# ZrrSkywalker/MonoDETR

Measured on AMD Instinct MI355X. Metric: training images/sec at B=8 per GPU, KITTI 384x1280, higher is better.
Workload: dtype bf16; 1 GPU; full MonoDETR training step (ResNet-50 + depth predictor + 3 enc / 3 dec layers, 550 train queries, 4 levels, criterion + AdamW) = BASELINE configs[2] (1 GPU) / configs[3] (DDP); global_batch=8, per_gpu_batch=8, image=3x384x1280, queries=50, precision=bf16, parallelism=dp1, grad_sync=none, prime_steps=12, launch=one hipGraph replay per iteration, cpu_affinity=NUMA node 0 of the GPU

## Files before the change

monodetr_amd/csrc/add_ln.hip:

```cpp
#include <hip/hip_runtime.h>
#include <hip/hip_bf16.h>
#include <stdint.h>

#include "add_ln.h"
#include "add_ln_math.h"

namespace mdetr {
namespace {

constexpr int kWavesLn = 4;
constexpr int kMaxBwdBlocks = 1024;

template <typename T> __device__ __forceinline__ float ld1(const T *p);
template <> __device__ __forceinline__ float ld1<float>(const float *p) { return *p; }
template <> __device__ __forceinline__ float ld1<__hip_bfloat16>(const __hip_bfloat16 *p) { return __bfloat162float(*p); }
template <typename T> __device__ __forceinline__ void st1(T *p, float v);
template <> __device__ __forceinline__ void st1<float>(float *p, float v) { *p = v; }
template <> __device__ __forceinline__ void st1<__hip_bfloat16>(__hip_bfloat16 *p, float v) { *p = __float2bfloat16(v); }

template <typename T, int E> struct alignas(sizeof(T) * E > 16 ? 16 : sizeof(T) * E) RowVec { T v[E]; };

template <typename T, int E> __device__ __forceinline__ void load_row(const T *p, float (&v)[E])
{
    const RowVec<T, E> t = *reinterpret_cast<const RowVec<T, E> *>(p);
#pragma unroll
    for (int i = 0; i < E; ++i) v[i] = ld1<T>(&t.v[i]);
}
template <typename T, int E> __device__ __forceinline__ void store_row(T *p, const float (&v)[E])
{
    RowVec<T, E> t;
#pragma unroll
    for (int i = 0; i < E; ++i) st1<T>(&t.v[i], v[i]);
    *reinterpret_cast<RowVec<T, E> *>(p) = t;
}

__device__ __forceinline__ float wave_sum(float v)
{
#pragma unroll
    for (int o = 32; o > 0; o >>= 1) v += __shfl_xor(v, o);
    return v;
}

template <typename T, typename PT, int E>
__global__ __launch_bounds__(kWavesLn * 64)
void add_ln_fwd_kernel(const T *__restrict__ a, const T *__restrict__ b, const PT *__restrict__ gamma,
                       const PT *__restrict__ beta, T *__restrict__ y, T *__restrict__ s, float *__restrict__ stats,
                       int64_t rows, float eps, uint32_t thresh, float keep_scale, uint64_t seed,
                       const uint64_t *__restrict__ seed_dev)
{
    constexpr int C = 64 * E;
    const int lane = threadIdx.x & 63, wave = threadIdx.x >> 6;
    const int64_t row = static_cast<int64_t>(blockIdx.x) * kWavesLn + wave;
    if (row >= rows) return;
    const uint64_t sd = seed + (seed_dev ? *seed_dev : 0ull);
    const int64_t at = row * C + lane * E;
    float v[E];
    load_row<T, E>(a + at, v);
    if (b) {
        float r[E];
        load_row<T, E>(b + at, r);
#pragma unroll
        for (int i = 0; i < E; ++i) {
            const bool keep = thresh == 0u || ln_hash(sd, static_cast<uint64_t>(at + i)) >= thresh;
            v[i] += keep ? r[i] * keep_scale : 0.f;
        }
        if (s) {
            store_row<T, E>(s + at, v);
#pragma unroll
            for (int i = 0; i < E; ++i) { T t; st1<T>(&t, v[i]); v[i] = ld1<T>(&t); }
        }
    }
    float sum = 0.f;
#pragma unroll
    for (int i = 0; i < E; ++i) sum += v[i];
    const float mean = wave_sum(sum) * (1.0f / C);
    float sq = 0.f;
#pragma unroll
    for (int i = 0; i < E; ++i) { const float d = v[i] - mean; sq += d * d; }
    const float rstd = 1.0f / sqrtf(wave_sum(sq) * (1.0f / C) + eps);
    float o[E];
#pragma unroll
    for (int i = 0; i < E; ++i) o[i] = (v[i] - mean) * rstd * ld1<PT>(gamma + lane * E + i) + ld1<PT>(beta + lane * E + i);
    store_row<T, E>(y + at, o);
    if (lane == 0) { stats[2 * row] = mean; stats[2 * row + 1] = rstd; }
}

template <typename T, typename PT, int E>
__global__ __launch_bounds__(kWavesLn * 64)
void add_ln_bwd_kernel(const T *__restrict__ dy, const T *__restrict__ s, const PT *__restrict__ gamma,
                       const float *__restrict__ stats, T *__restrict__ da, T *__restrict__ db,
                       float *__restrict__ partial, int64_t rows, uint32_t thresh, float keep_scale, uint64_t seed,
                       const uint64_t *__restrict__ seed_dev)
{
    constexpr int C = 64 * E;
    __shared__ float red[kWavesLn][2 * C];
    const int lane = threadIdx.x & 63, wave = threadIdx.x >> 6;
    const uint64_t sd = seed + (seed_dev ? *seed_dev : 0ull);
    float g[E], acc_g[E], acc_b[E];
#pragma unroll
    for (int i = 0; i < E; ++i) { g[i] = ld1<PT>(gamma + lane * E + i); acc_g[i] = 0.f; acc_b[i] = 0.f; }
    for (int64_t row = static_cast<int64_t>(blockIdx.x) * kWavesLn + wave; row < rows; row += static_cast<int64_t>(gridDim.x) * kWavesLn) {
        const int64_t at = row * C + lane * E;
        const float mean = stats[2 * row], rstd = stats[2 * row + 1];
        float d[E], x[E];
        load_row<T, E>(dy + at, d);
        load_row<T, E>(s + at, x);
        float s1 = 0.f, s2 = 0.f;
#pragma unroll
        for (int i = 0; i < E; ++i) {
            x[i] = (x[i] - mean) * rstd;
            acc_g[i] += d[i] * x[i];
            acc_b[i] += d[i];
            d[i] *= g[i];
            s1 += d[i];
            s2 += d[i] * x[i];
        }
        s1 = wave_sum(s1) * (1.0f / C);
        s2 = wave_sum(s2) * (1.0f / C);
        float o[E];
#pragma unroll
        for (int i = 0; i < E; ++i) o[i] = rstd * (d[i] - s1 - x[i] * s2);
        store_row<T, E>(da + at, o);
        if (db) {
#pragma unroll
            for (int i = 0; i < E; ++i) {
                const bool keep = thresh == 0u || ln_hash(sd, static_cast<uint64_t>(at + i)) >= thresh;
                o[i] = keep ? o[i] * keep_scale : 0.f;
            }
            store_row<T, E>(db + at, o);
        }
    }
#pragma unroll
    for (int i = 0; i < E; ++i) { red[wave][lane * E + i] = acc_g[i]; red[wave][C + lane * E + i] = acc_b[i]; }
    __syncthreads();
    for (int c = threadIdx.x; c < 2 * C; c += kWavesLn * 64)
        partial[static_cast<int64_t>(blockIdx.x) * 2 * C + c] = red[0][c] + red[1][c] + red[2][c] + red[3][c];
}

template <typename T, typename PT, int E>
hipError_t launch_fwd(const AddLnProblem &p, const void *a, const void *b, const void *gamma, const void *beta, void *y, void *s,
                      float *stats, hipStream_t st)
{
    const uint32_t thresh = b ? ln_threshold(p.dropout_p) : 0u;
    const float scale = p.dropout_p > 0.f ? 1.0f / (1.0f - p.dropout_p) : 1.0f;
    hipLaunchKernelGGL((add_ln_fwd_kernel<T, PT, E>), dim3(static_cast<unsigned>((p.rows + kWavesLn - 1) / kWavesLn)), dim3(kWavesLn * 64), 0, st,
                       static_cast<const T *>(a), static_cast<const T *>(b), static_cast<const PT *>(gamma), static_cast<const PT *>(beta),
                       static_cast<T *>(y), static_cast<T *>(s), stats,
                       p.rows, p.eps, thresh, scale, p.seed, p.seed_dev);
    return hipGetLastError();
}

template <typename T, typename PT, int E>
hipError_t launch_bwd(const AddLnProblem &p, const void *dy, const void *s, const void *gamma, const float *stats, void *da, void *db,
                      float *partial, hipStream_t st)
{
    const uint32_t thresh = db ? ln_threshold(p.dropout_p) : 0u;
    const float scale = p.dropout_p > 0.f ? 1.0f / (1.0f - p.dropout_p) : 1.0f;
    hipLaunchKernelGGL((add_ln_bwd_kernel<T, PT, E>), dim3(static_cast<unsigned>(add_ln_partial_rows(p.rows))), dim3(kWavesLn * 64), 0, st,
                       static_cast<const T *>(dy), static_cast<const T *>(s), static_cast<const PT *>(gamma), stats, static_cast<T *>(da),
                       static_cast<T *>(db), partial,
                       p.rows, thresh, scale, p.seed, p.seed_dev);
    return hipGetLastError();
}

}

int64_t add_ln_partial_rows(int64_t rows)
{
    const int64_t blocks = (rows + kWavesLn - 1) / kWavesLn;
    return blocks < 1 ? 1 : (blocks > kMaxBwdBlocks ? kMaxBwdBlocks : blocks);
}

template <int E>
hipError_t dispatch_fwd(const AddLnProblem &p, const void *a, const void *b, const void *gamma, const void *beta, void *y, void *s,
                        float *stats, hipStream_t st)
{
    using BF = __hip_bfloat16;
    if (p.io_dtype == 2) return p.param_dtype == 2 ? launch_fwd<BF, BF, E>(p, a, b, gamma, beta, y, s, stats, st) : launch_fwd<BF, float, E>(p, a, b, gamma, beta, y, s, stats, st);
    return p.param_dtype == 2 ? launch_fwd<float, BF, E>(p, a, b, gamma, beta, y, s, stats, st) : launch_fwd<float, float, E>(p, a, b, gamma, beta, y, s, stats, st);
}

template <int E>
hipError_t dispatch_bwd(const AddLnProblem &p, const void *dy, const void *s, const void *gamma, const float *stats, void *da, void *db,
                        float *partial, hipStream_t st)
{
    using BF = __hip_bfloat16;
    if (p.io_dtype == 2) return p.param_dtype == 2 ? launch_bwd<BF, BF, E>(p, dy, s, gamma, stats, da, db, partial, st) : launch_bwd<BF, float, E>(p, dy, s, gamma, stats, da, db, partial, st);
    return p.param_dtype == 2 ? launch_bwd<float, BF, E>(p, dy, s, gamma, stats, da, db, partial, st) : launch_bwd<float, float, E>(p, dy, s, gamma, stats, da, db, partial, st);
}

hipError_t add_ln_forward_launch(const AddLnProblem &p, const void *a, const void *b, const void *gamma, const void *beta,
                                 void *y, void *s, float *stats, hipStream_t st)
{
    if (p.rows == 0) return hipSuccess;
    switch (p.cols) {
    case 128: return dispatch_fwd<2>(p, a, b, gamma, beta, y, s, stats, st);
    case 256: return dispatch_fwd<4>(p, a, b, gamma, beta, y, s, stats, st);
    case 512: return dispatch_fwd<8>(p, a, b, gamma, beta, y, s, stats, st);
    default: return hipErrorNotSupported;
    }
}

hipError_t add_ln_backward_launch(const AddLnProblem &p, const void *dy, const void *s, const void *gamma, const float *stats,
                                  void *da, void *db, float *partial, hipStream_t st)
{
    if (p.rows == 0) return hipSuccess;
    switch (p.cols) {
    case 128: return dispatch_bwd<2>(p, dy, s, gamma, stats, da, db, partial, st);
    case 256: return dispatch_bwd<4>(p, dy, s, gamma, stats, da, db, partial, st);
    case 512: return dispatch_bwd<8>(p, dy, s, gamma, stats, da, db, partial, st);
    default: return hipErrorNotSupported;
    }
}

}
```

monodetr_amd/csrc/add_ln_math.h:

```cpp
#pragma once
#include <stdint.h>

#if defined(__HIPCC__)
#define MDETR_HD __host__ __device__ __forceinline__
#else
#define MDETR_HD inline
#endif

namespace mdetr {

MDETR_HD uint32_t ln_hash(uint64_t seed, uint64_t index)
{
    uint64_t z = index * 0x9E3779B97F4A7C15ull + seed;
    uint32_t x = static_cast<uint32_t>(z) ^ static_cast<uint32_t>(z >> 32);
    x ^= x >> 16;
    x *= 0x7FEB352Du;
    x ^= x >> 15;
    x *= 0x846CA68Bu;
    x ^= x >> 16;
    return x;
}

MDETR_HD uint32_t ln_threshold(float p)
{
    const double t = static_cast<double>(p) * 4294967296.0;
    return t >= 4294967295.0 ? 0xFFFFFFFFu : static_cast<uint32_t>(t);
}

}
```

monodetr_amd/csrc/conv_wgrad.hip:

```cpp
#include <hip/hip_runtime.h>
#include <stdint.h>
#include <stdlib.h>

#include <mdetr_wave.h>

#include "conv_wgrad.h"
#include "mdetr_tune.h"
#include "mdetr_transpose.h"
#include "mdetr_split.h"
#include "msda.h"

namespace mdetr {
namespace {

constexpr int kThreadsG = 512;
constexpr int kNB = 128, kCB = 64;
#ifndef MDETR_CONV_WGRAD_COLS
#define MDETR_CONV_WGRAD_COLS 16
#endif
constexpr int kRows = 8, kCols = MDETR_CONV_WGRAD_COLS;
constexpr int kDyStride = kCols + 1;

struct WgradGeom {
    ConvWgradDims d;
    int bands, ctiles, units, chunks, nblocks, cblocks;
};

template <int SI, int TS>
__global__ __launch_bounds__(kThreadsG)
void conv_wgrad_kernel(const __bf16 *__restrict__ x, const __bf16 *__restrict__ dy, float *__restrict__ part, const WgradGeom g)
{
    constexpr int P = TS == 3 ? 1 : 0;
    constexpr int XC = SI == 1 ? kCols + TS - 1 : (TS == 3 ? 2 * kCols + 1 : kCols);
    constexpr int XSTRIDE = XC | 1;
    constexpr int EVEN = kCols + 1;
    MDETR_DYNAMIC_LDS(unsigned char, wgrad_smem);
    bf16x8 *dyt = reinterpret_cast<bf16x8 *>(wgrad_smem);
    bf16x8 *xt = dyt + kNB * kDyStride;
    const ConvWgradDims &d = g.d;
    const int lane = threadIdx.x & 63, wave = threadIdx.x >> 6, half = lane >> 5, l31 = lane & 31;
    const int nsub = wave & 3, csub = wave >> 2;
    int id = blockIdx.x;
    const int chunk = id % g.chunks; id /= g.chunks;
    const int t = id % TS; id /= TS;
    const int cblk = id % g.cblocks; const int nblk = id / g.cblocks;
    const int n0 = nblk * kNB, c0 = cblk * kCB;

    f32x16 acc[TS];
#pragma unroll
    for (int e = 0; e < TS; ++e)
#pragma unroll
        for (int i = 0; i < 16; ++i) acc[e][i] = 0.f;
    const bool want_db = TS == 1 && d.DB != 0 && cblk == 0 && csub == 0;
    f32x16 accb;
#pragma unroll
    for (int i = 0; i < 16; ++i) accb[i] = 0.f;
    bf16x8 ones;
#pragma unroll
    for (int i = 0; i < 8; ++i) ones[i] = static_cast<__bf16>(1.0f);

    constexpr int CGX = (XC + 15) / 16;
    constexpr int WTASKS = 2 * CGX + 4 * (kCols / 16);
    constexpr int kWavesG = kThreadsG / 64;
    constexpr int ROUNDS = (WTASKS + kWavesG - 1) / kWavesG;
    constexpr int PF = ROUNDS <= 2 ? 2 : 1;
    bf16x8 stage[PF][ROUNDS][8];
    const mdetr_rsrc xr = make_rsrc(x, static_cast<unsigned>(static_cast<int64_t>(d.B) * d.H * d.W * d.C * 2));
    const mdetr_rsrc yr = make_rsrc(dy, static_cast<unsigned>(static_cast<int64_t>(d.B) * d.OH * d.OW * d.N * 2));
    const int ci = lane & 15, pi = lane >> 4;
    int t_rel[ROUNDS], t_ch[ROUNDS], t_dst[ROUNDS];
#pragma unroll
    for (int rd = 0; rd < ROUNDS; ++rd) {
        const int wt = wave + rd * kWavesG;
        if (wt < 2 * CGX) {
            const int slot = 16 * (wt >> 1) + ci, piece = 4 * (wt & 1) + pi;
            t_rel[rd] = slot >= XC ? -1 : (SI == 1 ? slot : (TS == 3 ? (slot < EVEN ? 2 * slot : 2 * (slot - EVEN) + 1) : 2 * slot));
            t_ch[rd] = (c0 + piece * 8) * 2;
            t_dst[rd] = piece * 8 * XSTRIDE + slot;
        } else {
            const int k = wt - 2 * CGX, col = 16 * (k >> 2) + ci, piece = 4 * (k & 3) + pi;
            t_rel[rd] = col;
            t_ch[rd] = (wt < WTASKS && n0 + piece * 8 < d.N) ? (n0 + piece * 8) * 2 : -1;
            t_dst[rd] = piece * 8 * kDyStride + col;
        }
    }
    auto fetch = [&](int u, bf16x8 (&st)[ROUNDS][8]) {
        const int ct = u % g.ctiles; u /= g.ctiles;
        const int band = u % g.bands; const int b = u / g.bands;
        const int r0 = band * kRows, q0 = ct * kCols;
#pragma unroll
        for (int rd = 0; rd < ROUNDS; ++rd) {
            const int wt = wave + rd * kWavesG;
            if (wt < 2 * CGX) {
                const int col = SI * q0 + t_rel[rd] - P;
                const unsigned lane_off = (t_rel[rd] >= 0 && col >= 0 && col < d.W) ? static_cast<unsigned>(col * d.C * 2 + t_ch[rd]) : kRsrcOob;
#pragma unroll
                for (int i = 0; i < 8; ++i) {
                    const int row = SI * (r0 + i) + t - P;
                    const bool ok = row >= 0 && row < d.H;
                    st[rd][i] = rsrc_load_bf16x8(xr, ok ? lane_off : kRsrcOob, ok ? static_cast<unsigned>((b * d.H + row) * d.W) * static_cast<unsigned>(d.C * 2) : 0u);
                }
            } else if (wt < WTASKS) {
                const int col = q0 + t_rel[rd];
                const unsigned lane_off = (col < d.OW && t_ch[rd] >= 0) ? static_cast<unsigned>(col * d.N * 2 + t_ch[rd]) : kRsrcOob;
#pragma unroll
                for (int i = 0; i < 8; ++i) {
                    const int row = r0 + i;
                    const bool ok = row < d.OH;
                    st[rd][i] = rsrc_load_bf16x8(yr, ok ? lane_off : kRsrcOob, ok ? static_cast<unsigned>((b * d.OH + row) * d.OW) * static_cast<unsigned>(d.N * 2) : 0u);
                }
            }
        }
    };
    auto commit = [&](const bf16x8 (&st)[ROUNDS][8]) {
#pragma unroll
        for (int rd = 0; rd < ROUNDS; ++rd) {
            const int wt = wave + rd * kWavesG;
            if (wt >= WTASKS) continue;
            bf16x8 tr[8];
            transpose8x8(st[rd], tr);
            if (wt < 2 * CGX) {
                if (16 * (wt >> 1) + ci < XC) {
#pragma unroll
                    for (int q = 0; q < 8; ++q) xt[t_dst[rd] + q * XSTRIDE] = tr[q];
                }
            } else {
#pragma unroll
                for (int q = 0; q < 8; ++q) dyt[t_dst[rd] + q * kDyStride] = tr[q];
            }
        }
    };
    auto products = [&]() {
        const bf16x8 *ap = dyt + (nsub * 32 + l31) * kDyStride + half;
        const bf16x8 *bp = xt + (csub * 32 + l31) * XSTRIDE;
#pragma unroll 4
        for (int ks = 0; ks < kCols / 2; ++ks) {
            const int q = 2 * ks + half;
            const bf16x8 a = ap[2 * ks];
#pragma unroll
            for (int e = 0; e < TS; ++e) {
                int slot;
                if (SI == 1) slot = q + e;
                else if (TS == 3) slot = (e & 1) ? EVEN + q : q + (e >> 1);
                else slot = q;
                acc[e] = mfma_bf16(a, bp[slot], acc[e]);
            }
            if (want_db) accb = mfma_bf16(a, ones, accb);
        }
    };

    int u = chunk;
    if (u < g.units) fetch(u, stage[0]);
    if (PF == 2 && u + g.chunks < g.units) fetch(u + g.chunks, stage[PF - 1]);
    while (u < g.units) {
#pragma unroll
        for (int s_ = 0; s_ < PF; ++s_) {
            if (u >= g.units) break;
            __syncthreads();
            commit(stage[s_]);
            const int nu = u + PF * g.chunks;
            if (nu < g.units) fetch(nu, stage[s_]);
            __syncthreads();
            products();
            u += g.chunks;
        }
    }

    const int c = c0 + csub * 32 + l31;
    float *pp = part + static_cast<int64_t>(chunk) * (static_cast<int64_t>(d.N) * TS * TS * d.C + (d.DB ? d.N : 0));
    if (want_db && l31 == 0) {
#pragma unroll
        for (int r = 0; r < 16; ++r) {
            const int n = n0 + nsub * 32 + (r & 3) + 8 * (r >> 2) + 4 * half;
            if (n < d.N) pp[static_cast<int64_t>(d.N) * d.C + n] = accb[r];
        }
    }
#pragma unroll
    for (int e = 0; e < TS; ++e)
#pragma unroll
        for (int r = 0; r < 16; ++r) {
            const int n = n0 + nsub * 32 + (r & 3) + 8 * (r >> 2) + 4 * half;
            if (n < d.N) pp[((static_cast<int64_t>(n) * TS + t) * TS + e) * d.C + c] = acc[e][r];
        }
}

template <int SI, int TS>
hipError_t launch(const void *x, const void *dy, float *part, WgradGeom g, hipStream_t st)
{
    constexpr int XC = SI == 1 ? kCols + TS - 1 : (TS == 3 ? 2 * kCols + 1 : kCols);
    constexpr size_t lds = (static_cast<size_t>(kNB) * kDyStride + static_cast<size_t>(kCB) * (XC | 1)) * 16;
    static_assert(lds <= 160 * 1024, "tile does not fit the LDS");
    auto kern = conv_wgrad_kernel<SI, TS>;
    static bool attr_set[64] = {};
    int dev_ = 0;
    if (hipGetDevice(&dev_) != hipSuccess) dev_ = -1;
    if (dev_ < 0 || dev_ >= 64 || !attr_set[dev_]) {
        const hipError_t e = hipFuncSetAttribute(reinterpret_cast<const void *>(kern), hipFuncAttributeMaxDynamicSharedMemorySize,
                                                 static_cast<int>(lds));
        if (e != hipSuccess) return e;
        if (dev_ >= 0 && dev_ < 64) attr_set[dev_] = true;
    }
    const int64_t blocks = static_cast<int64_t>(g.chunks) * TS * g.cblocks * g.nblocks;
    hipLaunchKernelGGL(kern, dim3(static_cast<unsigned>(blocks)), dim3(kThreadsG), lds, st, static_cast<const __bf16 *>(x),
                       static_cast<const __bf16 *>(dy), part, g);
    return hipGetLastError();
}

constexpr int kCols32 = 16;
constexpr int kDyStride32 = kCols32 + 1, kXC32 = kCols32 + 2, kXStride32 = kXC32 | 1;
constexpr int kDyPlane32 = kNB * kDyStride32, kXPlane32 = kCB * kXStride32;
constexpr size_t kLds32 = static_cast<size_t>(3) * (kDyPlane32 + kXPlane32) * 16;
static_assert(kLds32 == 162816 && kLds32 <= 160 * 1024, "three planes of the 128 x 64 tile: one workgroup per CU");

__global__ __launch_bounds__(kThreadsG)
void conv_wgrad_f32_kernel(const float *__restrict__ x, const float *__restrict__ dy, float *__restrict__ part, const WgradGeom g)
{
    constexpr int TS = 3;
    MDETR_DYNAMIC_LDS(unsigned char, wgrad32_smem);
    bf16x8 *dyt = reinterpret_cast<bf16x8 *>(wgrad32_smem);
    bf16x8 *xt = dyt + 3 * kDyPlane32;
    const ConvWgradDims &d = g.d;
    const int lane = threadIdx.x & 63, wave = threadIdx.x >> 6, half = lane >> 5, l31 = lane & 31;
    const int nsub = wave & 3, csub = wave >> 2;
    int id = blockIdx.x;
    const int chunk = id % g.chunks; id /= g.chunks;
    const int t = id % TS; id /= TS;
    const int cblk = id % g.cblocks; const int nblk = id / g.cblocks;
    const int n0 = nblk * kNB, c0 = cblk * kCB;

    f32x16 acc[TS];
#pragma unroll
    for (int e = 0; e < TS; ++e)
#pragma unroll
        for (int i = 0; i < 16; ++i) acc[e][i] = 0.f;

    constexpr int CGX = (kXC32 + 15) / 16;
    constexpr int WTASKS = 2 * CGX + 4 * (kCols32 / 16);
    static_assert(WTASKS == kThreadsG / 64, "one loading task per wave");
    bf16x8 stage[16];
    const mdetr_rsrc xr = make_rsrc(x, static_cast<unsigned>(static_cast<int64_t>(d.B) * d.H * d.W * d.C * 4));
    const mdetr_rsrc yr = make_rsrc(dy, static_cast<unsigned>(static_cast<int64_t>(d.B) * d.OH * d.OW * d.N * 4));
    const int ci = lane & 15, pi = lane >> 4;
    const bool is_x = wave < 2 * CGX;
    int t_rel, t_ch, t_dst;
    if (is_x) {
        const int slot = 16 * (wave >> 1) + ci, piece = 4 * (wave & 1) + pi;
        t_rel = slot >= kXC32 ? -1 : slot;
        t_ch = (c0 + piece * 8) * 4;
        t_dst = piece * 8 * kXStride32 + slot;
    } else {
        const int k = wave - 2 * CGX, col = 16 * (k >> 2) + ci, piece = 4 * (k & 3) + pi;
        t_rel = col;
        t_ch = n0 + piece * 8 < d.N ? (n0 + piece * 8) * 4 : -1;
        t_dst = piece * 8 * kDyStride32 + col;
    }
    auto fetch = [&](int u) {
        const int ct = u % g.ctiles; u /= g.ctiles;
        const int band = u % g.bands; const int b = u / g.bands;
        const int r0 = band * kRows, q0 = ct * kCols32;
        if (is_x) {
            const int col = q0 + t_rel - 1;
            const bool in = t_rel >= 0 && col >= 0 && col < d.W;
            const unsigned lane_off = in ? static_cast<unsigned>(col * d.C * 4 + t_ch) : 0u;
#pragma unroll
            for (int i = 0; i < 8; ++i) {
                const int row = r0 + i + t - 1;
                const bool ok = in && row >= 0 && row < d.H;
                const unsigned so = (row >= 0 && row < d.H) ? static_cast<unsigned>((b * d.H + row) * d.W) * static_cast<unsigned>(d.C * 4) : 0u;
                stage[2 * i] = rsrc_load_bf16x8(xr, ok ? lane_off : kRsrcOob, so);
                stage[2 * i + 1] = rsrc_load_bf16x8(xr, ok ? lane_off + 16u : kRsrcOob, so);
            }
        } else {
            const int col = q0 + t_rel;
            const bool in = col < d.OW && t_ch >= 0;
            const unsigned lane_off = in ? static_cast<unsigned>(col * d.N * 4 + t_ch) : 0u;
#pragma unroll
            for (int i = 0; i < 8; ++i) {
                const int row = r0 + i;
                const bool ok = in && row < d.OH;
                const unsigned so = row < d.OH ? static_cast<unsigned>((b * d.OH + row) * d.OW) * static_cast<unsigned>(d.N * 4) : 0u;
                stage[2 * i] = rsrc_load_bf16x8(yr, ok ? lane_off : kRsrcOob, so);
                stage[2 * i + 1] = rsrc_load_bf16x8(yr, ok ? lane_off + 16u : kRsrcOob, so);
            }
        }
    };
    auto commit = [&]() {
        bf16x8 pl[3][8];
#pragma unroll
        for (int i = 0; i < 8; ++i) {
#pragma unroll
            for (int s = 0; s < 2; ++s) {
                float f[4];
                __builtin_memcpy(f, &stage[2 * i + s], 16);
                bf16x4 h, m, l;
                split4(f, h, m, l);
#pragma unroll
                for (int j = 0; j < 4; ++j) { pl[0][i][4 * s + j] = h[j]; pl[1][i][4 * s + j] = m[j]; pl[2][i][4 * s + j] = l[j]; }
            }
        }
        if (is_x && t_rel < 0) return;
        bf16x8 *dst = is_x ? xt + t_dst : dyt + t_dst;
        const int stride = is_x ? kXStride32 : kDyStride32, plane = is_x ? kXPlane32 : kDyPlane32;
#pragma unroll
        for (int p = 0; p < 3; ++p) {
            bf16x8 tr[8];
            transpose8x8(pl[p], tr);
#pragma unroll
            for (int q = 0; q < 8; ++q) dst[p * plane + q * stride] = tr[q];
        }
    };
    auto products = [&]() {
        const bf16x8 *ap = dyt + (nsub * 32 + l31) * kDyStride32 + half;
        const bf16x8 *bp = xt + (csub * 32 + l31) * kXStride32 + half;
        constexpr int term_y[6] = {2, 0, 1, 1, 0, 0}, term_x[6] = {0, 2, 1, 0, 1, 0};
#pragma unroll 2
        for (int ks = 0; ks < kCols32 / 2; ++ks) {
            bf16x8 a[3], b[TS][3];
#pragma unroll
            for (int p = 0; p < 3; ++p) {
                a[p] = ap[p * kDyPlane32 + 2 * ks];
#pragma unroll
                for (int e = 0; e < TS; ++e) b[e][p] = bp[p * kXPlane32 + 2 * ks + e];
            }
#pragma unroll
            for (int k = 0; k < 6; ++k)
#pragma unroll
                for (int e = 0; e < TS; ++e) acc[e] = mfma_bf16(a[term_y[k]], b[e][term_x[k]], acc[e]);
        }
    };

    int u = chunk;
    if (u < g.units) fetch(u);
    while (u < g.units) {
        __syncthreads();
        commit();
        const int nu = u + g.chunks;
        if (nu < g.units) fetch(nu);
        __syncthreads();
        products();
        u = nu;
    }

    const int c = c0 + csub * 32 + l31;
    float *pp = part + static_cast<int64_t>(chunk) * (static_cast<int64_t>(d.N) * TS * TS * d.C);
#pragma unroll
// ... 51 lines not shown
#pragma unroll
    for (int e = 0; e < TS; ++e)
#pragma unroll
        for (int i = 0; i < 16; ++i) acc[e][i] = 0.f;

    constexpr int CGX = (kXCS2 + 7) / 8;
    static_assert(CGX + 1 == kThreadsS2 / 64, "one loading task per wave");
    bf16x8 stage[16];
    const mdetr_rsrc xr = make_rsrc(x, static_cast<unsigned>(static_cast<int64_t>(d.B) * d.H * d.W * d.C * 4));
    const mdetr_rsrc yr = make_rsrc(dy, static_cast<unsigned>(static_cast<int64_t>(d.B) * d.OH * d.OW * d.N * 4));
    const int ci = lane & 7, pi = lane >> 3;
    const bool is_x = wave < CGX;
    int t_rel, t_ch, t_dst;
    if (is_x) {
        const int slot = 8 * wave + ci;
        t_rel = slot >= kXCS2 ? -1 : (slot < kEvenS2 ? 2 * slot : 2 * (slot - kEvenS2) + 1);
        t_ch = (c0 + pi * 8) * 4;
        t_dst = pi * 8 * kXStrideS2 + slot;
    } else {
        t_rel = ci;
        t_ch = n0 + pi * 8 < d.N ? (n0 + pi * 8) * 4 : -1;
        t_dst = pi * 8 * kDyStrideS2 + ci;
    }
    auto fetch = [&](int u) {
        const int ct = u % g.ctiles; u /= g.ctiles;
        const int band = u % g.bands; const int b = u / g.bands;
        const int r0 = band * kRows, q0 = ct * kColsS2;
        if (is_x) {
            const int col = 2 * q0 + t_rel - 1;
            const bool in = t_rel >= 0 && col >= 0 && col < d.W;
            const unsigned lane_off = in ? static_cast<unsigned>(col * d.C * 4 + t_ch) : 0u;
#pragma unroll
            for (int i = 0; i < 8; ++i) {
                const int row = 2 * (r0 + i) + t - 1;
                const bool ok = in && row >= 0 && row < d.H;
                const unsigned so = (row >= 0 && row < d.H) ? static_cast<unsigned>((b * d.H + row) * d.W) * static_cast<unsigned>(d.C * 4) : 0u;
                stage[2 * i] = rsrc_load_bf16x8(xr, ok ? lane_off : kRsrcOob, so);
                stage[2 * i + 1] = rsrc_load_bf16x8(xr, ok ? lane_off + 16u : kRsrcOob, so);
            }
        } else {
            const int col = q0 + t_rel;
            const bool in = col < d.OW && t_ch >= 0;
            const unsigned lane_off = in ? static_cast<unsigned>(col * d.N * 4 + t_ch) : 0u;
#pragma unroll
            for (int i = 0; i < 8; ++i) {
                const int row = r0 + i;
                const bool ok = in && row < d.OH;
                const unsigned so = row < d.OH ? static_cast<unsigned>((b * d.OH + row) * d.OW) * static_cast<unsigned>(d.N * 4) : 0u;
                stage[2 * i] = rsrc_load_bf16x8(yr, ok ? lane_off : kRsrcOob, so);
                stage[2 * i + 1] = rsrc_load_bf16x8(yr, ok ? lane_off + 16u : kRsrcOob, so);
            }
        }
    };
    auto commit = [&]() {
        bf16x8 pl[3][8];
#pragma unroll
        for (int i = 0; i < 8; ++i) {
#pragma unroll
            for (int s = 0; s < 2; ++s) {
                float f[4];
                __builtin_memcpy(f, &stage[2 * i + s], 16);
                bf16x4 h, m, l;
                split4(f, h, m, l);
#pragma unroll
                for (int j = 0; j < 4; ++j) { pl[0][i][4 * s + j] = h[j]; pl[1][i][4 * s + j] = m[j]; pl[2][i][4 * s + j] = l[j]; }
            }
        }
        if (is_x && t_rel < 0) return;
        bf16x8 *dst = is_x ? xt + t_dst : dyt + t_dst;
        const int stride = is_x ? kXStrideS2 : kDyStrideS2, plane = is_x ? kXPlaneS2 : kDyPlaneS2;
#pragma unroll
        for (int p = 0; p < 3; ++p) {
            bf16x8 tr[8];
            transpose8x8(pl[p], tr);
#pragma unroll
            for (int q = 0; q < 8; ++q) dst[p * plane + q * stride] = tr[q];
        }
    };
    auto products = [&]() {
        const bf16x8 *ap = dyt + (nsub * 32 + l31) * kDyStrideS2 + half;
        const bf16x8 *bp = xt + (csub * 32 + l31) * kXStrideS2 + half;
        constexpr int term_y[6] = {2, 0, 1, 1, 0, 0}, term_x[6] = {0, 2, 1, 0, 1, 0};
#pragma unroll 2
        for (int ks = 0; ks < kColsS2 / 2; ++ks) {
            bf16x8 a[3], b[TS][3];
#pragma unroll
            for (int p = 0; p < 3; ++p) {
                a[p] = ap[p * kDyPlaneS2 + 2 * ks];
#pragma unroll
                for (int e = 0; e < TS; ++e)
                    b[e][p] = bp[p * kXPlaneS2 + 2 * ks + ((e & 1) ? kEvenS2 : (e >> 1))];
            }
#pragma unroll
            for (int k = 0; k < 6; ++k)
#pragma unroll
                for (int e = 0; e < TS; ++e) acc[e] = mfma_bf16(a[term_y[k]], b[e][term_x[k]], acc[e]);
        }
    };

    int u = chunk;
    if (u < g.units) fetch(u);
    while (u < g.units) {
        __syncthreads();
        commit();
        const int nu = u + g.chunks;
        if (nu < g.units) fetch(nu);
        __syncthreads();
        products();
        u = nu;
    }

    const int c = c0 + csub * 32 + l31;
    float *pp = part + static_cast<int64_t>(chunk) * (static_cast<int64_t>(d.N) * TS * TS * d.C);
#pragma unroll
    for (int e = 0; e < TS; ++e)
#pragma unroll
        for (int r = 0; r < 16; ++r) {
            const int n = n0 + nsub * 32 + (r & 3) + 8 * (r >> 2) + 4 * half;
            if (n < d.N) pp[((static_cast<int64_t>(n) * TS + t) * TS + e) * d.C + c] = acc[e][r];
        }
}

hipError_t launch_s2_f32(const void *x, const void *dy, float *part, WgradGeom g, hipStream_t st)
{
    auto kern = conv_wgrad_s2_f32_kernel;
    static bool attr_set[64] = {};
    int dev_ = 0;
    if (hipGetDevice(&dev_) != hipSuccess) dev_ = -1;
    if (dev_ < 0 || dev_ >= 64 || !attr_set[dev_]) {
        const hipError_t e = hipFuncSetAttribute(reinterpret_cast<const void *>(kern), hipFuncAttributeMaxDynamicSharedMemorySize,
                                                 static_cast<int>(kLdsS2));
        if (e != hipSuccess) return e;
        if (dev_ >= 0 && dev_ < 64) attr_set[dev_] = true;
    }
    const int64_t blocks = static_cast<int64_t>(g.chunks) * 3 * g.cblocks * g.nblocks;
    hipLaunchKernelGGL(kern, dim3(static_cast<unsigned>(blocks)), dim3(kThreadsS2), kLdsS2, st, static_cast<const float *>(x),
                       static_cast<const float *>(dy), part, g);
    return hipGetLastError();
}

WgradGeom geometry(const ConvWgradDims &d, int cols = kCols, int nb = kNB, int target = 256)
{
    WgradGeom g;
    g.d = d;
    g.bands = (d.OH + kRows - 1) / kRows;
    g.ctiles = (d.OW + cols - 1) / cols;
    g.units = d.B * g.bands * g.ctiles;
    g.nblocks = (d.N + nb - 1) / nb;
    g.cblocks = d.C / kCB;
    const int base = d.K * g.nblocks * g.cblocks;
    char tune_buf[16];
    if (const char *ev = tune_str("conv_wgrad_wgs", tune_buf, sizeof(tune_buf))) {
        const int f = atoi(ev);
        if (f >= 64 && f <= 8192) target = f;
    }
    int chunks = target / (base > 0 ? base : 1);
    if (chunks < 1) chunks = 1;
    if (chunks > g.units) chunks = g.units;
    g.chunks = chunks;
    return g;
}

}

bool conv_wgrad_supported(const ConvWgradDims &d, const void *x, const void *dy)
{
    const auto al = [](const void *p, uintptr_t a) { return (reinterpret_cast<uintptr_t>(p) & (a - 1)) == 0; };
    const bool shape = (d.K == 3 && (d.SI == 1 || d.SI == 2)) || (d.K == 1 && (d.SI == 2 || d.SI == 1));
    return shape && d.B > 0 && d.H > 0 && d.W > 0 && d.OH > 0 && d.OW > 0 && d.C > 0 && d.C % 64 == 0 && d.N > 0 && d.N % 32 == 0 &&
           al(x, 16) && al(dy, 16) && static_cast<int64_t>(d.N) * d.K * d.K * d.C < (1ll << 28) &&
           static_cast<int64_t>(d.B) * d.H * d.W * d.C < (1ll << 30) && static_cast<int64_t>(d.B) * d.OH * d.OW * d.N < (1ll << 30);
}

int conv_wgrad_chunks(const ConvWgradDims &d) { return geometry(d).chunks; }

hipError_t conv_wgrad_launch(const void *x, const void *dy, float *part, const ConvWgradDims &d, hipStream_t st)
{
    const WgradGeom g = geometry(d);
    ProfileScope prof(d.K == 1 && d.SI == 1 ? 11 : 9, conv_mflop(static_cast<int64_t>(d.B) * d.OH * d.OW, static_cast<int64_t>(d.C) * d.N * d.K * d.K), st,
                      2.0 * d.B * d.OH * d.OW * d.C * d.N * d.K * d.K / 1e6,
                      (2.0 * d.B * (static_cast<double>(d.H) * d.W * d.C + static_cast<double>(d.OH) * d.OW * d.N) + 4.0 * g.chunks * d.K * d.K * d.N * d.C) / 1e3);
    if (d.K == 3) return d.SI == 1 ? launch<1, 3>(x, dy, part, g, st) : launch<2, 3>(x, dy, part, g, st);
    return d.SI == 1 ? launch<1, 1>(x, dy, part, g, st) : launch<2, 1>(x, dy, part, g, st);
}

bool conv_wgrad_f32_supported(const ConvWgradDims &d, const void *x, const void *dy)
{
    const auto al = [](const void *p) { return (reinterpret_cast<uintptr_t>(p) & 15) == 0; };
    return d.K == 3 && d.SI == 1 && d.DB == 0 && d.B > 0 && d.H > 0 && d.W > 0 && d.OH == d.H && d.OW == d.W && d.C > 0 && d.C % 64 == 0 &&
           d.N > 0 && d.N % 32 == 0 && al(x) && al(dy) && static_cast<int64_t>(d.N) * 9 * d.C < (1ll << 28) &&
           static_cast<int64_t>(d.B) * d.H * d.W * d.C < (1ll << 29) && static_cast<int64_t>(d.B) * d.H * d.W * d.N < (1ll << 29);
}

int conv_wgrad_f32_chunks(const ConvWgradDims &d) { return geometry(d, kCols32).chunks; }

hipError_t conv_wgrad_f32_launch(const void *x, const void *dy, float *part, const ConvWgradDims &d, hipStream_t st)
{
    const WgradGeom g = geometry(d, kCols32);
    ProfileScope prof(9, conv_mflop(static_cast<int64_t>(d.B) * d.OH * d.OW, static_cast<int64_t>(d.C) * d.N * 9), st,
                      2.0 * d.B * d.OH * d.OW * d.C * d.N * 9 / 1e6,
                      (4.0 * d.B * (static_cast<double>(d.H) * d.W * d.C + static_cast<double>(d.OH) * d.OW * d.N) + 4.0 * g.chunks * 9 * d.N * d.C) / 1e3);
    return launch_f32(x, dy, part, g, st);
}

bool conv_wgrad_s2_f32_supported(const ConvWgradDims &d, const void *x, const void *dy)
{
    const auto al = [](const void *p) { return (reinterpret_cast<uintptr_t>(p) & 15) == 0; };
    return d.K == 3 && d.SI == 2 && d.DB == 0 && d.B > 0 && d.H > 0 && d.W > 0 && d.OH == (d.H - 1) / 2 + 1 && d.OW == (d.W - 1) / 2 + 1 &&
           d.C > 0 && d.C % 64 == 0 && d.N > 0 && d.N % 32 == 0 && al(x) && al(dy) && static_cast<int64_t>(d.N) * 9 * d.C < (1ll << 28) &&
           static_cast<int64_t>(d.B) * d.H * d.W * d.C < (1ll << 29) && static_cast<int64_t>(d.B) * d.OH * d.OW * d.N < (1ll << 29);
}

int conv_wgrad_s2_f32_chunks(const ConvWgradDims &d) { return geometry(d, kColsS2, kNBS2, 512).chunks; }

hipError_t conv_wgrad_s2_f32_launch(const void *x, const void *dy, float *part, const ConvWgradDims &d, hipStream_t st)
{
    const WgradGeom g = geometry(d, kColsS2, kNBS2, 512);
    ProfileScope prof(9, conv_mflop(static_cast<int64_t>(d.B) * d.OH * d.OW, static_cast<int64_t>(d.C) * d.N * 9), st,
                      2.0 * d.B * d.OH * d.OW * d.C * d.N * 9 / 1e6,
                      (4.0 * d.B * (static_cast<double>(d.H) * d.W * d.C + static_cast<double>(d.OH) * d.OW * d.N) + 4.0 * g.chunks * 9 * d.N * d.C) / 1e3);
    return launch_s2_f32(x, dy, part, g, st);
}

}
```

Before: 504.7 images/sec.

## Make add+LayerNorm kernels grid-stride with batched row loads and hoisted params

The forward add+LayerNorm kernel now runs on a capped grid-stride launch (256×8 blocks by default) and loads gamma/beta once per wave, using vector loads when they are aligned. Both forward and backward can batch R rows of loads ahead of compute, but R comes from a tuning knob whose default is 1. The dropout hash is computed incrementally per element run instead of with a full 64-bit multiply for each element. The aim is to cut launch and block-scheduling overhead, remove redundant parameter loads and lower hash arithmetic cost, at the price of less parallelism for small row counts.

Result: no change. 505.7 images/sec (median of 6 runs) (+0.2%).

```diff
diff --git a/monodetr_amd/csrc/add_ln.hip b/monodetr_amd/csrc/add_ln.hip
--- a/monodetr_amd/csrc/add_ln.hip
+++ b/monodetr_amd/csrc/add_ln.hip
@@ -4,12 +4,14 @@
 
 #include "add_ln.h"
 #include "add_ln_math.h"
+#include "mdetr_tune.h"
 
 namespace mdetr {
 namespace {
 
 constexpr int kWavesLn = 4;
 constexpr int kMaxBwdBlocks = 1024;
+constexpr int kFwdBlocksPerCu = 8;
 
 template <typename T> __device__ __forceinline__ float ld1(const T *p);
 template <> __device__ __forceinline__ float ld1<float>(const float *p) { return *p; }
@@ -20,9 +22,12 @@
 
 template <typename T, int E> struct alignas(sizeof(T) * E > 16 ? 16 : sizeof(T) * E) RowVec { T v[E]; };
 
-template <typename T, int E> __device__ __forceinline__ void load_row(const T *p, float (&v)[E])
-{
-    const RowVec<T, E> t = *reinterpret_cast<const RowVec<T, E> *>(p);
+template <typename T, int E> __device__ __forceinline__ RowVec<T, E> load_raw(const T *p)
+{
+    return *reinterpret_cast<const RowVec<T, E> *>(p);
+}
+template <typename T, int E> __device__ __forceinline__ void unpack_row(const RowVec<T, E> &t, float (&v)[E])
+{
 #pragma unroll
     for (int i = 0; i < E; ++i) v[i] = ld1<T>(&t.v[i]);
 }
@@ -33,6 +38,15 @@
     for (int i = 0; i < E; ++i) st1<T>(&t.v[i], v[i]);
     *reinterpret_cast<RowVec<T, E> *>(p) = t;
 }
+template <typename PT, int E> __device__ __forceinline__ void load_param(const PT *p, bool vec, float (&v)[E])
+{
+    if (vec) {
+        unpack_row<PT, E>(load_raw<PT, E>(p), v);
+    } else {
+#pragma unroll
+        for (int i = 0; i < E; ++i) v[i] = ld1<PT>(p + i);
+    }
+}
 
 __device__ __forceinline__ float wave_sum(float v)
 {
@@ -41,93 +55,147 @@
     return v;
 }
 
-template <typename T, typename PT, int E>
+template <int E> __device__ __forceinline__ void keep_run(uint64_t sd, int64_t at, uint32_t thresh, bool (&keep)[E])
+{
+    uint32_t h[E];
+    if (thresh != 0u) {
+        ln_hash_run<E>(sd, static_cast<uint64_t>(at), h);
+    } else {
+#pragma unroll
+        for (int i = 0; i < E; ++i) h[i] = 0u;
+    }
+#pragma unroll
+    for (int i = 0; i < E; ++i) keep[i] = h[i] >= thresh;
+}
+
+template <typename T, typename PT, int E, int R>
 __global__ __launch_bounds__(kWavesLn * 64)
 void add_ln_fwd_kernel(const T *__restrict__ a, const T *__restrict__ b, const PT *__restrict__ gamma,
                        const PT *__restrict__ beta, T *__restrict__ y, T *__restrict__ s, float *__restrict__ stats,
                        int64_t rows, float eps, uint32_t thresh, float keep_scale, uint64_t seed,
-                       const uint64_t *__restrict__ seed_dev)
+                       const uint64_t *__restrict__ seed_dev, int param_vec)
 {
     constexpr int C = 64 * E;
     const int lane = threadIdx.x & 63, wave = threadIdx.x >> 6;
-    const int64_t row = static_cast<int64_t>(blockIdx.x) * kWavesLn + wave;
-    if (row >= rows) return;
+    const int64_t stride = static_cast<int64_t>(gridDim.x) * kWavesLn;
+    const int64_t first = static_cast<int64_t>(blockIdx.x) * kWavesLn + wave;
+    if (first >= rows) return;
     const uint64_t sd = seed + (seed_dev ? *seed_dev : 0ull);
-    const int64_t at = row * C + lane * E;
-    float v[E];
-    load_row<T, E>(a + at, v);
-    if (b) {
-        float r[E];
-        load_row<T, E>(b + at, r);
-#pragma unroll
-        for (int i = 0; i < E; ++i) {
-            const bool keep = thresh == 0u || ln_hash(sd, static_cast<uint64_t>(at + i)) >= thresh;
-            v[i] += keep ? r[i] * keep_scale : 0.f;
-        }
-        if (s) {
-            store_row<T, E>(s + at, v);
-#pragma unroll
-            for (int i = 0; i < E; ++i) { T t; st1<T>(&t, v[i]); v[i] = ld1<T>(&t); }
-        }
-    }
-    float sum = 0.f;
-#pragma unroll
-    for (int i = 0; i < E; ++i) sum += v[i];
-    const float mean = wave_sum(sum) * (1.0f / C);
-    float sq = 0.f;
-#pragma unroll
-    for (int i = 0; i < E; ++i) { const float d = v[i] - mean; sq += d * d; }
-    const float rstd = 1.0f / sqrtf(wave_sum(sq) * (1.0f / C) + eps);
-    float o[E];
-#pragma unroll
-    for (int i = 0; i < E; ++i) o[i] = (v[i] - mean) * rstd * ld1<PT>(gamma + lane * E + i) + ld1<PT>(beta + lane * E + i);
-    store_row<T, E>(y + at, o);
-    if (lane == 0) { stats[2 * row] = mean; stats[2 * row + 1] = rstd; }
-}
-
-template <typename T, typename PT, int E>
+    float gm[E], bt[E];
+    load_param<PT, E>(gamma + lane * E, param_vec != 0, gm);
+    load_param<PT, E>(beta + lane * E, param_vec != 0, bt);
+    for (int64_t row0 = first; row0 < rows; row0 += stride * R) {
+        RowVec<T, E> ra[R], rb[R];
+#pragma unroll
+        for (int j = 0; j < R; ++j) {
+            const int64_t row = row0 + j * stride;
+            ra[j] = load_raw<T, E>(a + (row < rows ? row : rows - 1) * C + lane * E);
+        }
+        if (b) {
+#pragma unroll
+            for (int j = 0; j < R; ++j) {
+                const int64_t row = row0 + j * stride;
+                rb[j] = load_raw<T, E>(b + (row < rows ? row : rows - 1) * C + lane * E);
+            }
+        }
+#pragma unroll
+        for (int j = 0; j < R; ++j) {
+            const int64_t row = row0 + j * stride;
+            if (row < rows) {
+                const int64_t at = row * C + lane * E;
+                float v[E];
+                unpack_row<T, E>(ra[j], v);
+                if (b) {
+                    float r[E];
+                    unpack_row<T, E>(rb[j], r);
+                    bool keep[E];
+                    keep_run<E>(sd, at, thresh, keep);
+#pragma unroll
+                    for (int i = 0; i < E; ++i) v[i] += keep[i] ? r[i] * keep_scale : 0.f;
+                    if (s) {
+                        store_row<T, E>(s + at, v);
+#pragma unroll
+                        for (int i = 0; i < E; ++i) { T t; st1<T>(&t, v[i]); v[i] = ld1<T>(&t); }
+                    }
+                }
+                float sum = 0.f;
+#pragma unroll
+                for (int i = 0; i < E; ++i) sum += v[i];
+                const float mean = wave_sum(sum) * (1.0f / C);
+                float sq = 0.f;
+#pragma unroll
+                for (int i = 0; i < E; ++i) { const float d = v[i] - mean; sq += d * d; }
+                const float rstd = 1.0f / sqrtf(wave_sum(sq) * (1.0f / C) + eps);
+                float o[E];
+#pragma unroll
+                for (int i = 0; i < E; ++i) o[i] = (v[i] - mean) * rstd * gm[i] + bt[i];
+                store_row<T, E>(y + at, o);
+                if (lane == 0) { stats[2 * row] = mean; stats[2 * row + 1] = rstd; }
+            }
+        }
+    }
+}
+
+template <typename T, typename PT, int E, int R>
 __global__ __launch_bounds__(kWavesLn * 64)
 void add_ln_bwd_kernel(const T *__restrict__ dy, const T *__restrict__ s, const PT *__restrict__ gamma,
                        const float *__restrict__ stats, T *__restrict__ da, T *__restrict__ db,
                        float *__restrict__ partial, int64_t rows, uint32_t thresh, float keep_scale, uint64_t seed,
-                       const uint64_t *__restrict__ seed_dev)
+                       const uint64_t *__restrict__ seed_dev, int param_vec)
 {
     constexpr int C = 64 * E;
     __shared__ float red[kWavesLn][2 * C];
     const int lane = threadIdx.x & 63, wave = threadIdx.x >> 6;
+    const int64_t stride = static_cast<int64_t>(gridDim.x) * kWavesLn;
     const uint64_t sd = seed + (seed_dev ? *seed_dev : 0ull);
     float g[E], acc_g[E], acc_b[E];
-#pragma unroll
-    for (int i = 0; i < E; ++i) { g[i] = ld1<PT>(gamma + lane * E + i); acc_g[i] = 0.f; acc_b[i] = 0.f; }
-    for (int64_t row = static_cast<int64_t>(blockIdx.x) * kWavesLn + wave; row < rows; row += static_cast<int64_t>(gridDim.x) * kWavesLn) {
-        const int64_t at = row * C + lane * E;
-        const float mean = stats[2 * row], rstd = stats[2 * row + 1];
-        float d[E], x[E];
-        load_row<T, E>(dy + at, d);
-        load_row<T, E>(s + at, x);
-        float s1 = 0.f, s2 = 0.f;
-#pragma unroll
-        for (int i = 0; i < E; ++i) {
-            x[i] = (x[i] - mean) * rstd;
-            acc_g[i] += d[i] * x[i];
-            acc_b[i] += d[i];
-            d[i] *= g[i];
-            s1 += d[i];
-            s2 += d[i] * x[i];
-        }
-        s1 = wave_sum(s1) * (1.0f / C);
-        s2 = wave_sum(s2) * (1.0f / C);
-        float o[E];
-#pragma unroll
-        for (int i = 0; i < E; ++i) o[i] = rstd * (d[i] - s1 - x[i] * s2);
-        store_row<T, E>(da + at, o);
-        if (db) {
-#pragma unroll
-            for (int i = 0; i < E; ++i) {
-                const bool keep = thresh == 0u || ln_hash(sd, static_cast<uint64_t>(at + i)) >= thresh;
-                o[i] = keep ? o[i] * keep_scale : 0.f;
+    load_param<PT, E>(gamma + lane * E, param_vec != 0, g);
+#pragma unroll
+    for (int i = 0; i < E; ++i) { acc_g[i] = 0.f; acc_b[i] = 0.f; }
+    for (int64_t row0 = static_cast<int64_t>(blockIdx.x) * kWavesLn + wave; row0 < rows; row0 += stride * R) {
+        RowVec<T, E> rd[R], rx[R];
+        float mean_[R], rstd_[R];
+#pragma unroll
+        for (int j = 0; j < R; ++j) {
+            const int64_t row = row0 + j * stride, rc = row < rows ? row : rows - 1;
+            mean_[j] = stats[2 * rc];
+            rstd_[j] = stats[2 * rc + 1];
+            rd[j] = load_raw<T, E>(dy + rc * C + lane * E);
+            rx[j] = load_raw<T, E>(s + rc * C + lane * E);
+        }
+#pragma unroll
+        for (int j = 0; j < R; ++j) {
+            const int64_t row = row0 + j * stride;
+            if (row < rows) {
+                const int64_t at = row * C + lane * E;
+                const float mean = mean_[j], rstd = rstd_[j];
+                float d[E], x[E];
+                unpack_row<T, E>(rd[j], d);
+                unpack_row<T, E>(rx[j], x);
+                float s1 = 0.f, s2 = 0.f;
+#pragma unroll
+                for (int i = 0; i < E; ++i) {
+                    x[i] = (x[i] - mean) * rstd;
+                    acc_g[i] += d[i] * x[i];
+                    acc_b[i] += d[i];
+                    d[i] *= g[i];
+                    s1 += d[i];
+                    s2 += d[i] * x[i];
+                }
+                s1 = wave_sum(s1) * (1.0f / C);
+                s2 = wave_sum(s2) * (1.0f / C);
+                float o[E];
+#pragma unroll
+                for (int i = 0; i < E; ++i) o[i] = rstd * (d[i] - s1 - x[i] * s2);
+                store_row<T, E>(da + at, o);
+                if (db) {
+                    bool keep[E];
+                    keep_run<E>(sd, at, thresh, keep);
+#pragma unroll
+                    for (int i = 0; i < E; ++i) o[i] = keep[i] ? o[i] * keep_scale : 0.f;
+                    store_row<T, E>(db + at, o);
+                }
             }
-            store_row<T, E>(db + at, o);
         }
     }
 #pragma unroll
@@ -137,16 +205,56 @@
         partial[static_cast<int64_t>(blockIdx.x) * 2 * C + c] = red[0][c] + red[1][c] + red[2][c] + red[3][c];
 }
 
+int rows_per_trip()
+{
+    const int f = tune_int("add_ln_rows", 1);
+    return f == 2 || f == 4 ? f : 1;
+}
+
+template <typename PT, int E> bool param_aligned(const void *p)
+{
+    return (reinterpret_cast<uintptr_t>(p) & (alignof(RowVec<PT, E>) - 1)) == 0;
+}
+
+template <typename T, typename PT, int E, int R>
+hipError_t launch_fwd_r(const AddLnProblem &p, const void *a, const void *b, const void *gamma, const void *beta, void *y, void *s,
+                        float *stats, hipStream_t st)
+{
+    const uint32_t thresh = b ? ln_threshold(p.dropout_p) : 0u;
+    const float scale = p.dropout_p > 0.f ? 1.0f / (1.0f - p.dropout_p) : 1.0f;
+    int64_t grid = static_cast<int64_t>(256) * kFwdBlocksPerCu;
+    { const int f = tune_int("add_ln_grid", 0); if (f >= 1) grid = f; }
+    const int64_t blocks = (p.rows + kWavesLn - 1) / kWavesLn;
+    if (grid > blocks) grid = blocks;
+    const int pvec = param_aligned<PT, E>(gamma) && param_aligned<PT, E>(beta);
+    hipLaunchKernelGGL((add_ln_fwd_kernel<T, PT, E, R>), dim3(static_cast<unsigned>(grid)), dim3(kWavesLn * 64), 0, st,
+                       static_cast<const T *>(a), static_cast<const T *>(b), static_cast<const PT *>(gamma), static_cast<const PT *>(beta),
+                       static_cast<T *>(y), static_cast<T *>(s), stats,
+                       p.rows, p.eps, thresh, scale, p.seed, p.seed_dev, pvec);
+    return hipGetLastError();
+}
+
 template <typename T, typename PT, int E>
 hipError_t launch_fwd(const AddLnProblem &p, const void *a, const void *b, const void *gamma, const void *beta, void *y, void *s,
                       float *stats, hipStream_t st)
 {
-    const uint32_t thresh = b ? ln_threshold(p.dropout_p) : 0u;
+    switch (rows_per_trip()) {
+    case 1: return launch_fwd_r<T, PT, E, 1>(p, a, b, gamma, beta, y, s, stats, st);
+    case 2: return launch_fwd_r<T, PT, E, 2>(p, a, b, gamma, beta, y, s, stats, st);
+    default: return launch_fwd_r<T, PT, E, 4>(p, a, b, gamma, beta, y, s, stats, st);
+    }
+}
+
+template <typename T, typename PT, int E, int R>
+hipError_t launch_bwd_r(const AddLnProblem &p, const void *dy, const void *s, const void *gamma, const float *stats, void *da, void *db,
+                        float *partial, hipStream_t st)
+{
+    const uint32_t thresh = db ? ln_threshold(p.dropout_p) : 0u;
     const float scale = p.dropout_p > 0.f ? 1.0f / (1.0f - p.dropout_p) : 1.0f;
-    hipLaunchKernelGGL((add_ln_fwd_kernel<T, PT, E>), dim3(static_cast<unsigned>((p.rows + kWavesLn - 1) / kWavesLn)), dim3(kWavesLn * 64), 0, st,
-                       static_cast<const T *>(a), static_cast<const T *>(b), static_cast<const PT *>(gamma), static_cast<const PT *>(beta),
-                       static_cast<T *>(y), static_cast<T *>(s), stats,
-                       p.rows, p.eps, thresh, scale, p.seed, p.seed_dev);
+    hipLaunchKernelGGL((add_ln_bwd_kernel<T, PT, E, R>), dim3(static_cast<unsigned>(add_ln_partial_rows(p.rows))), dim3(kWavesLn * 64), 0, st,
+                       static_cast<const T *>(dy), static_cast<const T *>(s), static_cast<const PT *>(gamma), stats, static_cast<T *>(da),
+                       static_cast<T *>(db), partial,
+                       p.rows, thresh, scale, p.seed, p.seed_dev, static_cast<int>(param_aligned<PT, E>(gamma)));
     return hipGetLastError();
 }
 
@@ -154,13 +262,11 @@
 hipError_t launch_bwd(const AddLnProblem &p, const void *dy, const void *s, const void *gamma, const float *stats, void *da, void *db,
                       float *partial, hipStream_t st)
 {
-    const uint32_t thresh = db ? ln_threshold(p.dropout_p) : 0u;
-    const float scale = p.dropout_p > 0.f ? 1.0f / (1.0f - p.dropout_p) : 1.0f;
-    hipLaunchKernelGGL((add_ln_bwd_kernel<T, PT, E>), dim3(static_cast<unsigned>(add_ln_partial_rows(p.rows))), dim3(kWavesLn * 64), 0, st,
-                       static_cast<const T *>(dy), static_cast<const T *>(s), static_cast<const PT *>(gamma), stats, static_cast<T *>(da),
-                       static_cast<T *>(db), partial,
-                       p.rows, thresh, scale, p.seed, p.seed_dev);
-    return hipGetLastError();
+    switch (rows_per_trip()) {
+    case 1: return launch_bwd_r<T, PT, E, 1>(p, dy, s, gamma, stats, da, db, partial, st);
+    case 2: return launch_bwd_r<T, PT, E, 2>(p, dy, s, gamma, stats, da, db, partial, st);
+    default: return launch_bwd_r<T, PT, E, 4>(p, dy, s, gamma, stats, da, db, partial, st);
+    }
 }
 
 }
diff --git a/monodetr_amd/csrc/add_ln_math.h b/monodetr_amd/csrc/add_ln_math.h
--- a/monodetr_amd/csrc/add_ln_math.h
+++ b/monodetr_amd/csrc/add_ln_math.h
@@ -9,9 +9,10 @@
 
 namespace mdetr {
 
-MDETR_HD uint32_t ln_hash(uint64_t seed, uint64_t index)
+constexpr uint64_t kLnHashStep = 0x9E3779B97F4A7C15ull;
+
+MDETR_HD uint32_t ln_hash_mix(uint64_t z)
 {
-    uint64_t z = index * 0x9E3779B97F4A7C15ull + seed;
     uint32_t x = static_cast<uint32_t>(z) ^ static_cast<uint32_t>(z >> 32);
     x ^= x >> 16;
     x *= 0x7FEB352Du;
@@ -21,6 +22,21 @@
     return x;
 }
 
+MDETR_HD uint32_t ln_hash(uint64_t seed, uint64_t index)
+{
+    return ln_hash_mix(index * kLnHashStep + seed);
+}
+
+template <int E> MDETR_HD void ln_hash_run(uint64_t seed, uint64_t index, uint32_t (&h)[E])
+{
+    uint64_t z = index * kLnHashStep + seed;
+#pragma unroll
+    for (int i = 0; i < E; ++i) {
+        h[i] = ln_hash_mix(z);
+        z += kLnHashStep;
+    }
+}
+
 MDETR_HD uint32_t ln_threshold(float p)
 {
     const double t = static_cast<double>(p) * 4294967296.0;
```

## Double-buffer LDS tiles in stride-2 3x3 conv weight-gradient kernel

Applied to the files above, without the earlier changes.

For the 3x3 stride-2 weight-gradient kernel, the change adds a second LDS buffer so that committing the next tile overlaps with MFMA products on the current one. This replaces two barriers per tile with one. It also trims the k-steps on partial right-edge column tiles, and adds a mode in which half the waves commit before computing so the two kinds of work are staggered. The cost is LDS use above 130KB, which limits residency to one workgroup per CU. Two tiles are staged in registers, which adds register pressure.

Result: no change. 510.5 images/sec before, 512.7 images/sec after (median of 6 runs) (+0.4%).

```diff
diff --git a/monodetr_amd/csrc/conv_wgrad.hip b/monodetr_amd/csrc/conv_wgrad.hip
--- a/monodetr_amd/csrc/conv_wgrad.hip
+++ b/monodetr_amd/csrc/conv_wgrad.hip
@@ -15,18 +15,16 @@
 
 constexpr int kThreadsG = 512;
 constexpr int kNB = 128, kCB = 64;
-#ifndef MDETR_CONV_WGRAD_COLS
-#define MDETR_CONV_WGRAD_COLS 16
-#endif
-constexpr int kRows = 8, kCols = MDETR_CONV_WGRAD_COLS;
+constexpr int kRows = 8, kCols = 16;
 constexpr int kDyStride = kCols + 1;
 
 struct WgradGeom {
     ConvWgradDims d;
     int bands, ctiles, units, chunks, nblocks, cblocks;
+    int mode;
 };
 
-template <int SI, int TS>
+template <int SI, int TS, bool PIPE>
 __global__ __launch_bounds__(kThreadsG)
 void conv_wgrad_kernel(const __bf16 *__restrict__ x, const __bf16 *__restrict__ dy, float *__restrict__ part, const WgradGeom g)
 {
@@ -34,9 +32,9 @@
     constexpr int XC = SI == 1 ? kCols + TS - 1 : (TS == 3 ? 2 * kCols + 1 : kCols);
     constexpr int XSTRIDE = XC | 1;
     constexpr int EVEN = kCols + 1;
+    constexpr int BUF = kNB * kDyStride + kCB * XSTRIDE;
     MDETR_DYNAMIC_LDS(unsigned char, wgrad_smem);
-    bf16x8 *dyt = reinterpret_cast<bf16x8 *>(wgrad_smem);
-    bf16x8 *xt = dyt + kNB * kDyStride;
+    bf16x8 *const lds = reinterpret_cast<bf16x8 *>(wgrad_smem);
     const ConvWgradDims &d = g.d;
     const int lane = threadIdx.x & 63, wave = threadIdx.x >> 6, half = lane >> 5, l31 = lane & 31;
     const int nsub = wave & 3, csub = wave >> 2;
@@ -63,8 +61,8 @@
     constexpr int WTASKS = 2 * CGX + 4 * (kCols / 16);
     constexpr int kWavesG = kThreadsG / 64;
     constexpr int ROUNDS = (WTASKS + kWavesG - 1) / kWavesG;
-    constexpr int PF = ROUNDS <= 2 ? 2 : 1;
-    bf16x8 stage[PF][ROUNDS][8];
+    static_assert(ROUNDS <= 2, "two tiles wait in registers: 32 registers per round and tile");
+    bf16x8 stage[2][ROUNDS][8];
     const mdetr_rsrc xr = make_rsrc(x, static_cast<unsigned>(static_cast<int64_t>(d.B) * d.H * d.W * d.C * 2));
     const mdetr_rsrc yr = make_rsrc(dy, static_cast<unsigned>(static_cast<int64_t>(d.B) * d.OH * d.OW * d.N * 2));
     const int ci = lane & 15, pi = lane >> 4;
@@ -112,7 +110,8 @@
             }
         }
     };
-    auto commit = [&](const bf16x8 (&st)[ROUNDS][8]) {
+    auto commit = [&](const bf16x8 (&st)[ROUNDS][8], int buf) {
+        bf16x8 *dyt = lds + buf * BUF, *xt = dyt + kNB * kDyStride;
 #pragma unroll
         for (int rd = 0; rd < ROUNDS; ++rd) {
             const int wt = wave + rd * kWavesG;
@@ -130,39 +129,76 @@
             }
         }
     };
-    auto products = [&]() {
+    auto kstep = [&](const bf16x8 *ap, const bf16x8 *bp, int ks) {
+        const int q = 2 * ks + half;
+        const bf16x8 a = ap[2 * ks];
+#pragma unroll
+        for (int e = 0; e < TS; ++e) {
+            int slot;
+            if (SI == 1) slot = q + e;
+            else if (TS == 3) slot = (e & 1) ? EVEN + q : q + (e >> 1);
+            else slot = q;
+            acc[e] = mfma_bf16(a, bp[slot], acc[e]);
+        }
+        if (want_db) accb = mfma_bf16(a, ones, accb);
+    };
+    auto products = [&](int buf, int nks) {
+        const bf16x8 *dyt = lds + buf * BUF, *xt = dyt + kNB * kDyStride;
         const bf16x8 *ap = dyt + (nsub * 32 + l31) * kDyStride + half;
         const bf16x8 *bp = xt + (csub * 32 + l31) * XSTRIDE;
+        if (nks == kCols / 2) {
 #pragma unroll 4
-        for (int ks = 0; ks < kCols / 2; ++ks) {
-            const int q = 2 * ks + half;
-            const bf16x8 a = ap[2 * ks];
-#pragma unroll
-            for (int e = 0; e < TS; ++e) {
-                int slot;
-                if (SI == 1) slot = q + e;
-                else if (TS == 3) slot = (e & 1) ? EVEN + q : q + (e >> 1);
-                else slot = q;
-                acc[e] = mfma_bf16(a, bp[slot], acc[e]);
-            }
-            if (want_db) accb = mfma_bf16(a, ones, accb);
-        }
-    };
-
-    int u = chunk;
-    if (u < g.units) fetch(u, stage[0]);
-    if (PF == 2 && u + g.chunks < g.units) fetch(u + g.chunks, stage[PF - 1]);
-    while (u < g.units) {
-#pragma unroll
-        for (int s_ = 0; s_ < PF; ++s_) {
-            if (u >= g.units) break;
-            __syncthreads();
-            commit(stage[s_]);
-            const int nu = u + PF * g.chunks;
-            if (nu < g.units) fetch(nu, stage[s_]);
-            __syncthreads();
-            products();
-            u += g.chunks;
+            for (int ks = 0; ks < kCols / 2; ++ks) kstep(ap, bp, ks);
+        } else {
+            for (int ks = 0; ks < nks; ++ks) kstep(ap, bp, ks);
+        }
+    };
+
+    if constexpr (PIPE) {
+        const int nt = chunk < g.units ? (g.units - chunk + g.chunks - 1) / g.chunks : 0;
+        const bool early = g.mode != 0 && wave_uniform(csub) != 0;
+        auto live_ksteps = [&](int j) {
+            const int left = d.OW - ((chunk + j * g.chunks) % g.ctiles) * kCols;
+            return left >= kCols ? kCols / 2 : (left + 1) >> 1;
+        };
+        if (nt > 0) fetch(chunk, stage[0]);
+        if (nt > 1) fetch(chunk + g.chunks, stage[1]);
+        if (nt > 0) {
+            commit(stage[0], 0);
+            if (nt > 2) fetch(chunk + 2 * g.chunks, stage[0]);
+        }
+        __syncthreads();
+        for (int j = 0; j < nt; j += 2) {
+#pragma unroll
+            for (int s_ = 0; s_ < 2; ++s_) {
+                const int jj = j + s_;
+                if (jj >= nt) break;
+                const int nks = live_ksteps(jj);
+                if (!early) products(s_, nks);
+                if (jj + 1 < nt) {
+                    commit(stage[s_ ^ 1], s_ ^ 1);
+                    if (jj + 3 < nt) fetch(chunk + (jj + 3) * g.chunks, stage[s_ ^ 1]);
+                }
+                if (early) products(s_, nks);
+                __syncthreads();
+            }
+        }
+    } else {
+        int u = chunk;
+        if (u < g.units) fetch(u, stage[0]);
+        if (u + g.chunks < g.units) fetch(u + g.chunks, stage[1]);
+        while (u < g.units) {
+#pragma unroll
+            for (int s_ = 0; s_ < 2; ++s_) {
+                if (u >= g.units) break;
+                __syncthreads();
+                commit(stage[s_], 0);
+                const int nu = u + 2 * g.chunks;
+                if (nu < g.units) fetch(nu, stage[s_]);
+                __syncthreads();
+                products(0, kCols / 2);
+                u += g.chunks;
+            }
         }
     }
 
@@ -187,10 +223,13 @@
 template <int SI, int TS>
 hipError_t launch(const void *x, const void *dy, float *part, WgradGeom g, hipStream_t st)
 {
+    constexpr bool PIPE = SI == 2 && TS == 3;
     constexpr int XC = SI == 1 ? kCols + TS - 1 : (TS == 3 ? 2 * kCols + 1 : kCols);
-    constexpr size_t lds = (static_cast<size_t>(kNB) * kDyStride + static_cast<size_t>(kCB) * (XC | 1)) * 16;
-    static_assert(lds <= 160 * 1024, "tile does not fit the LDS");
-    auto kern = conv_wgrad_kernel<SI, TS>;
+    constexpr size_t lds = (PIPE ? 2 : 1) * (static_cast<size_t>(kNB) * kDyStride + static_cast<size_t>(kCB) * (XC | 1)) * 16;
+    static_assert(lds == (SI == 1 ? (TS == 3 ? 54272 : 52224) : (TS == 3 ? 137216 : 52224)),
+                  "dYt 128 x 17 and Xt 64 x 19 / 33 / 17 slots of 16 bytes; two such buffers at 3x3 / stride 2");
+    static_assert(lds <= 160 * 1024, "the buffers do not fit the LDS");
+    auto kern = conv_wgrad_kernel<SI, TS, PIPE>;
     static bool attr_set[64] = {};
     int dev_ = 0;
     if (hipGetDevice(&dev_) != hipSuccess) dev_ = -1;
@@ -548,7 +587,12 @@
     char tune_buf[16];
     if (const char *ev = tune_str("conv_wgrad_wgs", tune_buf, sizeof(tune_buf))) {
         const int f = atoi(ev);
-        if (f >= 64 && f <= 8192) target = f;
+        if (f >= 1 && f <= 8192) target = f;
+    }
+    g.mode = 1;
+    if (const char *ev = tune_str("conv_wgrad_mode", tune_buf, sizeof(tune_buf))) {
+        const int f = atoi(ev);
+        if (f == 0 || f == 1) g.mode = f;
     }
     int chunks = target / (base > 0 ? base : 1);
     if (chunks < 1) chunks = 1;
```
